# theovincent/i-DQN

Hardware: NVIDIA B200
Metric: i-DQN grad steps/sec (NatureCNN K=5, batch 32) (higher is better)
Workload: dtype f32

## Files before the change

i-dqn_b200/csrc/dense_wgrad_tma.cuh:

```cuda
#pragma once
#include "common.cuh"
#include "tc_core.cuh"
#include "tma_core.cuh"

namespace dwt {
using namespace tc;
typedef __nv_bfloat16 bf16;

constexpr int NTHREADS = 608;
constexpr int STAGES = 3;
constexpr int TM = 8;
constexpr int TN = 32;
constexpr int TO = 128;
constexpr int CB = 4;
constexpr uint32_t TILE_F32 = TM * CB * TO * 4;
constexpr uint32_t X_PLANE = 32 * TN * 2;
constexpr uint32_t STAGE_BYTES = 3 * TILE_F32 + 2 * X_PLANE;
constexpr uint32_t DY_CB = 2 * 2 * 32 * 128;
constexpr uint32_t DY_BYTES = CB * DY_CB;
constexpr uint32_t BAR_OFF = STAGES * STAGE_BYTES + DY_BYTES;
constexpr uint32_t SMEM_TOTAL = BAR_OFF + 256 + 1024;
constexpr uint32_t TMEM_COLS = 512;

struct Args {
  int heads, tile0, ntiles;
  int I, O;
  const int32_t* count;
  float lr, b1, b2, eps;
  float* grad;
  unsigned long long stream_policy;
  int64_t stride, w_off;
  int tl_id;
};

__device__ __forceinline__ void tma_store_3d(const CUtensorMap* map, uint32_t src, int c0, int c1, int c2) {
  asm volatile("cp.async.bulk.tensor.3d.global.shared::cta.bulk_group [%0, {%2, %3, %4}], [%1];" ::"l"(map), "r"(src),
               "r"(c0), "r"(c1), "r"(c2)
               : "memory");
}
__device__ __forceinline__ void bulk_commit() { asm volatile("cp.async.bulk.commit_group;" ::: "memory"); }
template <int N>
__device__ __forceinline__ void bulk_wait_read() {
  asm volatile("cp.async.bulk.wait_group.read %0;" ::"n"(N) : "memory");
}
__device__ __forceinline__ void bulk_wait_all() { asm volatile("cp.async.bulk.wait_group 0;" ::: "memory"); }
__device__ __forceinline__ void epi_bar_sync() { asm volatile("bar.sync 1, 512;" ::: "memory"); }

__global__ void __launch_bounds__(NTHREADS, 1)
dense_wgrad_adam_kernel(const __grid_constant__ CUtensorMap mapX_hi, const __grid_constant__ CUtensorMap mapX_lo,
                        const __grid_constant__ CUtensorMap mapDy_hi, const __grid_constant__ CUtensorMap mapDy_lo,
                        const __grid_constant__ CUtensorMap mapW, const __grid_constant__ CUtensorMap mapM,
                        const __grid_constant__ CUtensorMap mapV, const Args p) {
  extern __shared__ uint8_t smem_raw[];
  const uint32_t base = (smem_u32(smem_raw) + 1023u) & ~1023u;
  uint8_t* smem = smem_raw + (base - smem_u32(smem_raw));
  uint64_t* bars = reinterpret_cast<uint64_t*>(smem + BAR_OFF);
  uint64_t* full = bars;
  uint64_t* empty = bars + 4;
  uint64_t* acc_full = bars + 8;
  uint64_t* acc_empty = bars + 10;
  uint64_t* a_full = bars + 12;
  uint64_t* a_empty = bars + 13;
  uint64_t* ready = bars + 14;
  __shared__ uint32_t tmem_base_s;

  const int tid = threadIdx.x, warp = tid >> 5, lane = tid & 31;
  ktl_begin(p.tl_id);
  if (tid == 0) {
    for (int i = 0; i < STAGES; ++i) mbar_init(&full[i], 1), mbar_init(&empty[i], 1), mbar_init(&ready[i], 1);
    for (int i = 0; i < 2; ++i) mbar_init(&acc_full[i], 1), mbar_init(&acc_empty[i], 16);
    mbar_init(a_full, 1), mbar_init(a_empty, 1);
    fence_mbar_init();
  }
  if (warp == 1) tmem_alloc(&tmem_base_s, TMEM_COLS);
  fence_proxy_async_smem();
  tcgen05_before_sync();
  __syncthreads();
  tcgen05_after_sync();
  const uint32_t tmem = tmem_base_s;

  const int n_items = p.heads * p.ntiles;
  const int i0 = (int)((int64_t)blockIdx.x * n_items / gridDim.x), i1 = (int)((int64_t)(blockIdx.x + 1) * n_items / gridDim.x);
  const uint32_t as = base + STAGES * STAGE_BYTES;

  if (warp == 0) {
    if (elect_one()) {
      int st = 0, ai = 0, last_z = -1;
      uint32_t ph = 0;
      for (int it = i0; it < i1; ++it) {
        const int z = it / p.ntiles, row0 = (p.tile0 + it % p.ntiles) * TM;
        if (z != last_z) {
          last_z = z;
          mbar_wait(a_empty, (ai & 1) ^ 1);
          tma::expect_tx(a_full, DY_BYTES);
          for (int g = 0; g < 2 * CB; ++g) {
            const uint32_t dst = as + (g >> 1) * DY_CB + (g & 1) * 4096;
            tma::load_3d(dst, &mapDy_hi, a_full, g * 64, 0, z);
            tma::load_3d(dst + 8192, &mapDy_lo, a_full, g * 64, 0, z);
          }
          ++ai;
        }
        mbar_wait(&empty[st], ph ^ 1);
        tma::expect_tx(&full[st], STAGE_BYTES);
        const uint32_t s0 = base + st * STAGE_BYTES;
        tma::load_3d(s0 + 3 * TILE_F32, &mapX_hi, &full[st], row0, 0, z);
        tma::load_3d(s0 + 3 * TILE_F32 + X_PLANE, &mapX_lo, &full[st], row0, 0, z);
        for (int hb = 0; hb < 2; ++hb) {
          tma::load_3d_hint(s0 + hb * (TILE_F32 / 2), &mapW, &full[st], hb * 256, row0, z, p.stream_policy);
          tma::load_3d_hint(s0 + TILE_F32 + hb * (TILE_F32 / 2), &mapM, &full[st], hb * 256, row0, z, p.stream_policy);
          tma::load_3d_hint(s0 + 2 * TILE_F32 + hb * (TILE_F32 / 2), &mapV, &full[st], hb * 256, row0, z, p.stream_policy);
        }
        if (++st == STAGES) st = 0, ph ^= 1;
      }
    }
  } else if (warp == 1) {
    if (elect_one()) {
      const uint32_t idesc2 = make_idesc_bf16(128, 2 * TN, true, true);
      const uint32_t idesc1 = make_idesc_bf16(128, TN, true, true);
      const uint32_t a_hi32 = tma::desc_hi32(1024, tma::LT_SW128), b_hi32 = tma::desc_hi32(512, tma::LT_SW64);
      int st = 0, ai = 0, ti = 0, last_z = -1;
      uint32_t ph = 0;
      for (int it = i0; it < i1; ++it, ++ti) {
        const int z = it / p.ntiles;
        if (z != last_z) {
          last_z = z;
          mbar_wait(a_full, ai & 1);
          ++ai;
        }
        const int ab = ti & 1;
        mbar_wait(&acc_empty[ab], ((ti >> 1) & 1) ^ 1);
        mbar_wait(&full[st], ph);
        tcgen05_after_sync();
        const uint32_t xh = tma::desc_lo32(base + st * STAGE_BYTES + 3 * TILE_F32, X_PLANE);
#pragma unroll
        for (int cbk = 0; cbk < CB; ++cbk) {
          const uint32_t d = tmem + (uint32_t)ab * (CB * 2 * TN) + cbk * 2 * TN;
          const uint32_t ah = tma::desc_lo32(as + cbk * DY_CB, 4096), al = tma::desc_lo32(as + cbk * DY_CB + 8192, 4096);
          tma::mma_bf16_split<false>(d, ah, a_hi32, xh, b_hi32, idesc2);
          tma::mma_bf16_split<true>(d, al, a_hi32, xh, b_hi32, idesc1);
          tma::mma_bf16_split<true>(d, ah + 128, a_hi32, xh + 64, b_hi32, idesc2);
          tma::mma_bf16_split<true>(d, al + 128, a_hi32, xh + 64, b_hi32, idesc1);
        }
        mma_commit(&acc_full[ab]);
        if (it + 1 == i1 || (it + 1) / p.ntiles != z) mma_commit(a_empty);
        if (++st == STAGES) st = 0, ph ^= 1;
      }
    }
  } else if (warp == 18) {
    if (elect_one()) {
      int st = 0;
      uint32_t ph = 0;
      for (int it = i0; it < i1; ++it) {
        const int z = it / p.ntiles, row0 = (p.tile0 + it % p.ntiles) * TM;
        mbar_wait(&ready[st], ph);
        const uint32_t src = base + st * STAGE_BYTES;
        for (int hb = 0; hb < 2; ++hb) {
          tma::store_3d_hint(&mapW, src + hb * (TILE_F32 / 2), hb * 256, row0, z, p.stream_policy);
          tma::store_3d_hint(&mapM, src + TILE_F32 + hb * (TILE_F32 / 2), hb * 256, row0, z, p.stream_policy);
          tma::store_3d_hint(&mapV, src + 2 * TILE_F32 + hb * (TILE_F32 / 2), hb * 256, row0, z, p.stream_policy);
        }
        bulk_commit();
        bulk_wait_read<0>();
        tma::arrive(&empty[st]);
        if (++st == STAGES) st = 0, ph ^= 1;
      }
      bulk_wait_all();
    }
  } else {
    const int q = warp & 3, o = q * 32 + lane, cbk = (warp - 2) >> 2;
    int st = 0, ti = 0, last_z = -1;
    uint32_t ph = 0;
    AdamCoef ac;
    for (int it = i0; it < i1; ++it, ++ti) {
      const int z = it / p.ntiles, row0 = (p.tile0 + it % p.ntiles) * TM;
      if (z != last_z) {
        last_z = z;
        ac = adam_coef(p.b1, p.b2, p.lr, p.eps, p.count[z]);
      }
      const int ab = ti & 1;
      mbar_wait(&acc_full[ab], (ti >> 1) & 1);
      mbar_wait(&full[st], ph);
      tcgen05_after_sync();
      float g[16];
      {
        const uint32_t taddr = tmem + ((uint32_t)(q * 32) << 16) + (uint32_t)ab * (CB * 2 * TN) + cbk * 2 * TN;
        float g2[16];
        tmem_ld16_nowait(taddr, g);
        tmem_ld16_nowait(taddr + TN, g2);
        tmem_ld_wait();
#pragma unroll
        for (int e = 0; e < TM; ++e) g[e] += g2[e];
      }
      tcgen05_before_sync();
      __syncwarp();
      if (lane == 0) tma::arrive(&acc_empty[ab]);
      float* sW = reinterpret_cast<float*>(smem + st * STAGE_BYTES + (cbk >> 1) * (TILE_F32 / 2)) + (cbk & 1) * 128 + o;
      float* sM = sW + TILE_F32 / 4;
      float* sV = sM + TILE_F32 / 4;
      const int64_t gb = (int64_t)z * p.stride + p.w_off + (int64_t)row0 * p.O + cbk * 128 + o;
      float P[TM], M[TM], V[TM];
#pragma unroll
      for (int e = 0; e < TM; ++e) P[e] = sW[e * 256], M[e] = sM[e * 256], V[e] = sV[e * 256];
#pragma unroll
      for (int e = 0; e < TM; ++e) {
        adam_elem(ac, g[e], P[e], M[e], V[e]);
        sW[e * 256] = P[e], sM[e * 256] = M[e], sV[e * 256] = V[e];
      }
      fence_proxy_async_smem();
      epi_bar_sync();
      if (tid == 64) tma::arrive(&ready[st]);
      if (p.grad) {
#pragma unroll
        for (int e = 0; e < TM; ++e) p.grad[gb + (int64_t)e * p.O] = g[e];
      }
      if (++st == STAGES) st = 0, ph ^= 1;
    }
  }
  tcgen05_before_sync();
  __syncthreads();
  ktl_end(p.tl_id);
  if (warp == 1) tmem_dealloc(tmem, TMEM_COLS);
}

}
```

i-dqn_b200/csrc/img_host.cuh:

```cuda
#pragma once
#include "conv_img.cuh"
#include "dense_stream.cuh"
#include "dense_wgrad_tma.cuh"

struct ImgHost {
  img::Geom g[IDQN_IMG_LAYERS];
  img::TapsArgs fwd[IDQN_IMG_LAYERS], dg[IDQN_IMG_LAYERS];
  img::WgradArgs wg[IDQN_IMG_LAYERS];
  img::S2dArgs s2d;
  img::ChainArgs chain;
  int chain_on;
  int dense_on;
  alignas(64) CUtensorMap fmapWf[2], fmapWd, dmapX[2], dmapDy[2];
  alignas(64) CUtensorMap wmapX[2], wmapP[3];
  int wgrad_tma_on;
  dense::Args dfwd, ddg;
  float* dpart;
  int* dtickets;
};

static int img_chunks(int rows, int* chunk_rows, int* rows_alloc) {
  const int n = (rows + 255) / 256;
  int cr = ((rows + n - 1) / n + 7) / 8 * 8;
  *chunk_rows = cr;
// ... 471 lines not shown
  CK(cudaGetLastError());
  mark(h, dgrad ? "img_dgrad_L%d" : "img_fwd_L%d", li);
  return IDQN_OK;
}

static int img_launch_chain_fwd(idqn_handle* h) {
  ImgHost* H = (ImgHost*)h->img_host;
  img::ChainArgs c = H->chain;
  c.a.tl_id = tl_next(h);
  const img::ChainSmem L = img::chain_smem(c);
  const int per = (c.a.n_units + h->sm_avail - 1) / h->sm_avail;
  const int grid = (c.a.n_units + per - 1) / per;
  CK(img_set_smem(img::conv_chain_fwd_kernel, L.total));
  CK(launch_pdl(h->pdl, img::conv_chain_fwd_kernel, dim3(grid), dim3(img::NTHREADS), L.total, h->stream, h->il[1].mapX[0],
                h->il[1].mapX[1], h->il[1].mapW[0], h->il[1].mapW[1], h->il[2].mapW[0], h->il[2].mapW[1], c));
  CK(cudaGetLastError());
  mark(h, "img_fwd_chain_L%d", 1);
  return IDQN_OK;
}

static int img_launch_wgrad(idqn_handle* h, int li, int a_planes) {
  ImgHost* H = (ImgHost*)h->img_host;
  img::WgradArgs a = H->wg[li];
  a.debug = img_debug_on("wgrad", li);
  a.tl_id = tl_next(h);
  const ImgLayerState& S = h->il[li];
  const img::WgradSmem L = img::wgrad_smem(a, a_planes);
  const int grid = a.heads * a.groups * a.tsplit;
  if (a_planes == 1) {
    CK(img_set_smem(img::conv_wgrad_kernel<1>, L.total));
    CK(launch_pdl(h->pdl, img::conv_wgrad_kernel<1>, dim3(grid), dim3(img::WG_THREADS), L.total, h->stream, S.mapXw[0], S.mapXw[1],
                  S.mapZw[0], S.mapZw[1], a));
  } else {
    CK(img_set_smem(img::conv_wgrad_kernel<2>, L.total));
    CK(launch_pdl(h->pdl, img::conv_wgrad_kernel<2>, dim3(grid), dim3(img::WG_THREADS), L.total, h->stream, S.mapXw[0], S.mapXw[1],
                  S.mapZw[0], S.mapZw[1], a));
  }
  CK(cudaGetLastError());
  mark(h, "img_wgrad_L%d", li);
  return IDQN_OK;
}

static int dense_launch(idqn_handle* h, bool dgrad, bool z_dst, int unit0 = -1, int n_units = -1) {
  ImgHost* H = (ImgHost*)h->img_host;
  dense::Args a = dgrad ? H->ddg : H->dfwd;
  if (unit0 >= 0) a.unit0 = unit0, a.n_units = n_units;
  a.tl_id = unit0 >= 0 ? -1 : tl_next(h);
  const int li = IDQN_IMG_LAYERS;
  a.debug = img_debug_on(dgrad ? "ddgrad" : "dfwd", li);
  if (dgrad && z_dst) {
    const img::Geom& pg = H->g[li - 1];
    a.yh = h->il[li - 1].dz_hi, a.yl = h->il[li - 1].dz_lo;
    a.zP = pg.P, a.zW = pg.OW, a.zC = pg.OC, a.zOff = pg.T - 1, a.zRows = pg.ZRa, a.zstride = h->il[li - 1].dz_net_stride;
  }
  a.keep_heads = l2_keep_heads(h);
  const dense::Smem L = dense::smem_layout(a);
  int grid = std::min(a.n_units, h->sm_count);
  {
    static const bool rounds_env = !getenv("IDQN_NO_ROUNDS");
    if (rounds_env && unit0 < 0) {
      const int per = (a.n_units + grid - 1) / grid;
      grid = (a.n_units + per - 1) / per;
    }
  }
  if (dgrad) {
    CK(img_set_smem(dense::dense_stream_kernel<1>, L.total));
    CK(launch_pdl(h->pdl, dense::dense_stream_kernel<1>, dim3(grid), dim3(dense::NTHREADS), L.total, h->stream,
                  H->fmapWd, H->fmapWd, H->dmapDy[0], H->dmapDy[1], a));
  } else {
    CK(img_set_smem(dense::dense_stream_kernel<0>, L.total));
    CK(launch_pdl(h->pdl, dense::dense_stream_kernel<0>, dim3(grid), dim3(dense::NTHREADS), L.total, h->stream,
                  H->fmapWf[0], H->fmapWf[1], H->dmapX[0], H->dmapX[1], a));
  }
  CK(cudaGetLastError());
  mark(h, dgrad ? "dense_dgrad_L%d" : "dense_fwd_L%d", li);
  return IDQN_OK;
}

static int dense_wgrad_launch(idqn_handle* h, int tile0, int ntiles, bool keep_grads) {
  ImgHost* H = (ImgHost*)h->img_host;
  const Layer& l = h->layers[IDQN_IMG_LAYERS];
  dwt::Args a;
  a.heads = h->K, a.tile0 = tile0, a.ntiles = ntiles;
  a.I = l.g.Kd, a.O = l.g.OC;
  a.count = h->count;
  a.lr = h->cfg.learning_rate, a.b1 = 0.9f, a.b2 = 0.999f, a.eps = h->cfg.adam_eps;
  a.grad = keep_grads ? h->grad : nullptr;
  static const int sp = getenv("IDQN_L2_STREAM") ? atoi(getenv("IDQN_L2_STREAM")) : 0;
  a.stream_policy = sp == 0 ? tma::L2_EVICT_NORMAL : (sp == 2 ? tma::L2_EVICT_LAST : tma::L2_EVICT_FIRST);
  a.stride = h->stride, a.w_off = l.w_off;
  a.tl_id = tl_next(h);
  const int grid = std::min(a.heads * a.ntiles, h->sm_avail);
  CK(img_set_smem(dwt::dense_wgrad_adam_kernel, dwt::SMEM_TOTAL));
  CK(launch_pdl(0, dwt::dense_wgrad_adam_kernel, dim3(grid), dim3(dwt::NTHREADS), dwt::SMEM_TOTAL, h->stream, H->wmapX[0],
                H->wmapX[1], H->dmapDy[0], H->dmapDy[1], H->wmapP[0], H->wmapP[1], H->wmapP[2], a));
  CK(cudaGetLastError());
  mark(h, "dense_wgrad_adam_L%d", IDQN_IMG_LAYERS);
  return IDQN_OK;
}

static int img_rebuild_activation(idqn_handle* h, int net, int layer) {
  ImgHost* H = (ImgHost*)h->img_host;
  const img::Geom& g = H->g[layer];
  img::PlaneDst d = H->fwd[layer].dst;
  float* out = h->act + (int64_t)net * h->act_stride + h->layers[layer].act_off;
  const int64_t total = (int64_t)h->B * g.OH * g.OW * g.OC;
  img::planes_to_f32_kernel<<<(int)std::min<int64_t>((total + 255) / 256, 4096), 256, 0, h->stream>>>(d, net, h->B, g.OH, g.OW,
                                                                                                 g.OC, out);
  CK(cudaGetLastError());
  return IDQN_OK;
}
```

i-dqn_b200/csrc/net.cu:

```cuda
#include "common.cuh"
#include "gemm_simt.cuh"
#include "gemm_tc.cuh"
#include "sm_partition.cuh"

#include <algorithm>
#include <cmath>

static thread_local char g_err[512] = "";
void idqn_set_error(const char* fmt, ...) {
  va_list ap;
  va_start(ap, fmt);
  vsnprintf(g_err, sizeof(g_err), fmt, ap);
  va_end(ap);
}
extern "C" const char* idqn_last_error(void) { return g_err; }
extern "C" int idqn_version(void) { return 100; }

static void same_pad(int in, int k, int s, int* out, int* lo) {
  *out = (in + s - 1) / s;
  int total = std::max((*out - 1) * s + k - in, 0);
  *lo = total / 2;
}

static void finish_geom(ConvGeom& g) {
// ... 862 lines not shown
    tcg::TcDgradConv p;
    p.g = l.g;
    p.dyh = h->dact_hi + l.act_off, p.dyl = h->dact_lo + l.act_off, p.dystride = h->act_stride;
    p.wh = wh, p.wl = wl;
    p.w_off = l.w_off;
    p.xact = h->act + prev.act_off, p.dx = h->dact + prev.act_off;
    p.mask = mask, p.add = add;
    p.dxh = h->dact_hi + prev.act_off, p.dxl = h->dact_lo + prev.act_off, p.xstride = h->act_stride;
    p.ncls = S * S, p.JH = JH, p.JW = JW;
    p.d_jwoc = FastDiv(JW * l.g.OC);
    p.K = JH * JW * l.g.OC;
    p.NT = round16(l.g.IC);
    p.nstage = tcg::pick_stages(2, p.NT, (p.K + 31) / 32);
    for (int cl = 0; cl < p.ncls; ++cl) {
      p.cls_niy[cl] = cls_niy[cl], p.cls_nix[cl] = cls_nix[cl];
      p.cls_d_n[cl] = FastDiv(std::max(cls_niy[cl] * cls_nix[cl], 1));
      p.cls_d_nix[cl] = FastDiv(std::max(cls_nix[cl], 1));
    }
    dim3 grid((maxM + 127) / 128, 1, K * p.ncls);
    CK((tcg::launch_tc<false, false, 2, false, true, false>(p, grid, h->part, h->tickets, h->stream)));
    mark(h, "tc_dgrad_L%d", li);
    return IDQN_OK;
  }
  DgradProb p;
  p.g = l.g;
  p.dy = h->dact + l.act_off;
  p.dystride = h->act_stride;
  p.w = NetPtr{h->online, h->online, h->stride, h->stride, K};
  p.w_off = l.w_off;
  p.xact = h->act + prev.act_off;
  p.mask = mask, p.add = add;
  p.dx = h->dact + prev.act_off;
  p.dxh = h->dact_hi + prev.act_off, p.dxl = h->dact_lo + prev.act_off;
  p.xstride = h->act_stride;
  p.nz = K;
  p.S = 1;
  p.ncls = S * S;
  p.JH = JH, p.JW = JW;
  p.d_jwoc = FastDiv(JW * l.g.OC);
  p.N = l.g.IC;
  p.K = JH * JW * l.g.OC;
  p.kchunk = p.K;
  for (int cl = 0; cl < p.ncls; ++cl) {
    p.cls_niy[cl] = cls_niy[cl], p.cls_nix[cl] = cls_nix[cl];
    p.cls_d_n[cl] = FastDiv(std::max(cls_niy[cl] * cls_nix[cl], 1));
    p.cls_d_nix[cl] = FastDiv(std::max(cls_nix[cl], 1));
  }
  p.M = maxM;
  CK((launch_gemm_simt<true, true>(p, K * p.ncls, h->part, h->tickets, h->stream)));
  mark(h, "dgrad_L%d", li);
  return IDQN_OK;
}

static int launch_adam_ranges(idqn_handle* h, int64_t off_a, int64_t len_a, bool a_from_partials, int64_t off_b,
                              int64_t len_b, bool coresident = false) {
  len_a = std::max<int64_t>(len_a, 0), len_b = std::max<int64_t>(len_b, 0);
  if (len_a + len_b <= 0) return IDQN_OK;
  const int64_t n4a = len_a / 4, n4b = len_b / 4;
  const int cap = h->sm_count * 8;
  const int bt = coresident ? 128 : 256;
  const int ba = n4a ? (int)std::min<int64_t>((n4a + bt - 1) / bt, cap) : 0;
  const int bb = n4b ? (int)std::min<int64_t>((n4b + bt - 1) / bt, cap) : 0;
  if (coresident) {
    static bool carve_set = false;
    if (!carve_set) {
      CK(cudaFuncSetAttribute(adam_kernel, cudaFuncAttributePreferredSharedMemoryCarveout, cudaSharedmemCarveoutMaxShared));
      carve_set = true;
    }
  }
  dim3 grid(std::max(ba + bb, 1), h->K);
  const bool keep = (h->cfg.flags & IDQN_F_KEEP_GRADS) != 0;
  CK(launch_pdl(h->pdl && !coresident, adam_kernel, grid, dim3(bt), 0, h->stream, (float4*)h->online, (const float4*)h->grad, (float4*)h->mu, (float4*)h->nu,
                                           (uint2*)h->won_hi, (uint2*)h->won_lo, h->count, h->stride / 4, off_a / 4, n4a, ba,
                                           off_b / 4, n4b, h->cfg.learning_rate, 0.9f, 0.999f, h->cfg.adam_eps,
                                           a_from_partials ? (const float4*)h->wpart : nullptr, h->wgroups, h->wspan / 4,
                                           (a_from_partials && keep) ? (float4*)h->grad : nullptr, tl_next(h)));
  mark(h, "adam_%d", 0);
  return IDQN_OK;
}

static int dense_update_ctas(const idqn_handle* h) {
  static const int env = getenv("IDQN_WG_OVERLAP") ? atoi(getenv("IDQN_WG_OVERLAP")) : -1;
  if (h->update_ctas_set > 0) return std::min(h->sm_count, h->update_ctas_set - 1);
  return env >= 0 ? env : (h->K <= 10 ? std::min(h->sm_count, (116 + 13 * h->K) / 2 * h->sm_count / 148) : 0);
}

static int enqueue_learn_step(idqn_handle* h, int x_u8, bool dry = false, int64_t* ws_part = nullptr,
                              int* ws_tick = nullptr) {
  const int K = h->K, L = h->n_layers, B = h->B;
  h->n_launch = 0;
  const bool use_img = h->img_on && x_u8 && !dry;
  const int n_img = use_img ? IDQN_IMG_LAYERS : 0;
  if (!dry) h->img_last = use_img;
  const bool in_planes = use_tc(h) && (tc_conv_ok(h->layers[0]) || tc_dense_ok(h, h->layers[0]));
  if (use_img) {
    int rc = img_launch_s2d(h, x_u8);
    if (rc) return rc;
    const bool chain = ((ImgHost*)h->img_host)->chain_on && (h->cfg.flags & IDQN_F_CHAIN);
    for (int li = 0; li < n_img; ++li) {
      if (chain && li == 1) {
        rc = img_launch_chain_fwd(h);
        li = 2;
      } else {
        rc = img_launch_taps(h, li, false, li == 0 ? 1 : 2);
      }
      if (rc) return rc;
    }
  } else if (in_planes && !dry) {
    int rc = launch_input_planes(h, x_u8, B, 1);
    if (rc) return rc;
  }
  const int64_t in_full = (int64_t)B * h->in_elems;
  const bool use_dense = h->img_on && !dry && ((ImgHost*)h->img_host)->dense_on;
  for (int li = n_img; li < L - 1; ++li) {
    if (use_dense && li == IDQN_IMG_LAYERS) {
      int rc = dense_launch(h, false, false);
      if (rc) return rc;
      continue;
    }
    FwdIO io;
    int nh = 1;
    if (li == 0) {
      io.x = NetPtr{h->s, h->s2, 0, 0, K};
      io.xh = NetPtr{h->in_hi, h->in_hi + in_full, 0, 0, K};
      io.xl = NetPtr{h->in_lo, h->in_lo + in_full, 0, 0, K};
      nh = K;
    } else {
      const int64_t o = h->layers[li - 1].act_off;
      io.x = NetPtr{h->act + o, h->act + o, h->act_stride, h->act_stride, 2 * K};
      io.xh = NetPtr{h->act_hi + o, h->act_hi + o, h->act_stride, h->act_stride, 2 * K};
      io.xl = NetPtr{h->act_lo + o, h->act_lo + o, h->act_stride, h->act_stride, 2 * K};
    }
    io.w = NetPtr{h->online, h->target, h->stride, h->stride, K};
    io.wh = NetPtr{h->won_hi, h->wtg_hi, h->stride, h->stride, K};
    io.wl = NetPtr{h->won_lo, h->wtg_lo, h->stride, h->stride, K};
    const int64_t o = h->layers[li].act_off;
    io.y = h->act + o, io.yh = h->act_hi + o, io.yl = h->act_lo + o, io.ystride = h->act_stride;
    if (h->layers[li].kind == IDQN_LAYER_POOL) {
      if (dry) continue;
      int rc = launch_pool_fwd(h, li, 2 * K, B, h->act + h->layers[li - 1].act_off, h->act + o, h->act_stride, true);
      if (rc) return rc;
      continue;
    }
    int rc = launch_fwd_layer(h, li, 2 * K, nh, B, io, li == 0 ? x_u8 : 0, h->layers[li].relu_out, dry, ws_part, ws_tick);
    if (rc) return rc;
  }
  if (!dry) {
    const Layer& l = h->layers[L - 1];
    HeadArgs a;
    if (L >= 2) {
      const float* hid = h->act + h->layers[L - 2].act_off;
      a.hid = NetPtr{hid, hid, h->act_stride, h->act_stride, 2 * K};
      a.dhid = h->dact + h->layers[L - 2].act_off;
      a.dhid_hi = h->dact_hi + h->layers[L - 2].act_off, a.dhid_lo = h->dact_lo + h->layers[L - 2].act_off;
      a.relu_mask = 1;
    } else {
      REQUIRE(!x_u8, "a network without hidden layers needs float32 inputs");
      a.hid = NetPtr{h->s, h->s2, 0, 0, K};
      a.dhid = nullptr;
      a.dhid_hi = a.dhid_lo = nullptr;
      a.relu_mask = 0;
    }
    a.H = l.g.Kd, a.A = h->A, a.B = B, a.K = K;
    a.online = h->online, a.target = h->target;
    a.stride = h->stride, a.w_off = l.w_off, a.b_off = l.b_off;
    a.action = h->action, a.reward = h->reward, a.terminal = h->terminal;
    a.gamma_n = h->cfg.gamma_n;
// ... 953 lines not shown
```

i-dqn_b200/csrc/tc_core.cuh:

```cuda
#pragma once
#include <cuda_bf16.h>
#include <cuda_runtime.h>
#include <stdint.h>

namespace tc {

__device__ __forceinline__ uint32_t smem_u32(const void* p) { return (uint32_t)__cvta_generic_to_shared(p); }

__device__ __forceinline__ void mbar_init(uint64_t* bar, uint32_t count) {
  asm volatile("mbarrier.init.shared::cta.b64 [%0], %1;" ::"r"(smem_u32(bar)), "r"(count) : "memory");
}
__device__ __forceinline__ void fence_mbar_init() { asm volatile("fence.mbarrier_init.release.cluster;" ::: "memory"); }
__device__ __forceinline__ bool mbar_try_wait(uint64_t* bar, uint32_t parity) {
  uint32_t ok;
  asm volatile(
      "{\n"
      ".reg .pred p;\n"
      "mbarrier.try_wait.parity.shared::cta.b64 p, [%1], %2;\n"
      "selp.u32 %0, 1, 0, p;\n"
      "}\n"
      : "=r"(ok)
      : "r"(smem_u32(bar)), "r"(parity)
      : "memory");
  return ok != 0;
}
__device__ __forceinline__ void mbar_wait(uint64_t* bar, uint32_t parity) {
  uint32_t spins = 0;
  while (!mbar_try_wait(bar, parity)) {
    if (++spins > (1u << 24)) __trap();
  }
}

__device__ __forceinline__ bool elect_one() {
  uint32_t pred = 0, laneid = 0;
  asm volatile(
      "{\n"
      ".reg .b32 %%rx;\n"
      ".reg .pred %%px;\n"
      "     elect.sync %%rx|%%px, %2;\n"
      "@%%px mov.s32 %1, 1;\n"
      "     mov.s32 %0, %%rx;\n"
      "}\n"
      : "+r"(laneid), "+r"(pred)
      : "r"(0xFFFFFFFF));
  return pred != 0;
}

__device__ __forceinline__ void fence_proxy_async_smem() { asm volatile("fence.proxy.async.shared::cta;" ::: "memory"); }
__device__ __forceinline__ void tcgen05_before_sync() { asm volatile("tcgen05.fence::before_thread_sync;" ::: "memory"); }
__device__ __forceinline__ void tcgen05_after_sync() { asm volatile("tcgen05.fence::after_thread_sync;" ::: "memory"); }

__device__ __forceinline__ void tmem_alloc(uint32_t* smem_dst, uint32_t ncols) {
  __syncwarp();
  asm volatile("tcgen05.alloc.cta_group::1.sync.aligned.shared::cta.b32 [%0], %1;" ::"r"(smem_u32(smem_dst)), "r"(ncols)
               : "memory");
  asm volatile("tcgen05.relinquish_alloc_permit.cta_group::1.sync.aligned;" ::: "memory");
}
__device__ __forceinline__ void tmem_dealloc(uint32_t taddr, uint32_t ncols) {
  __syncwarp();
  asm volatile("tcgen05.dealloc.cta_group::1.sync.aligned.b32 %0, %1;" ::"r"(taddr), "r"(ncols) : "memory");
}
__device__ __forceinline__ void tmem_ld16(uint32_t taddr, float* v) {
  uint32_t r[16];
  __syncwarp();
  asm volatile(
      "tcgen05.ld.sync.aligned.32x32b.x16.b32 {%0,%1,%2,%3,%4,%5,%6,%7,%8,%9,%10,%11,%12,%13,%14,%15}, [%16];"
      : "=r"(r[0]), "=r"(r[1]), "=r"(r[2]), "=r"(r[3]), "=r"(r[4]), "=r"(r[5]), "=r"(r[6]), "=r"(r[7]), "=r"(r[8]),
        "=r"(r[9]), "=r"(r[10]), "=r"(r[11]), "=r"(r[12]), "=r"(r[13]), "=r"(r[14]), "=r"(r[15])
      : "r"(taddr)
      : "memory");
  asm volatile("tcgen05.wait::ld.sync.aligned;" ::: "memory");
#pragma unroll
  for (int i = 0; i < 16; ++i) v[i] = __uint_as_float(r[i]);
}

__device__ __forceinline__ void tmem_ld16_nowait(uint32_t taddr, float* v) {
  uint32_t r[16];
  __syncwarp();
  asm volatile(
      "tcgen05.ld.sync.aligned.32x32b.x16.b32 {%0,%1,%2,%3,%4,%5,%6,%7,%8,%9,%10,%11,%12,%13,%14,%15}, [%16];"
      : "=r"(r[0]), "=r"(r[1]), "=r"(r[2]), "=r"(r[3]), "=r"(r[4]), "=r"(r[5]), "=r"(r[6]), "=r"(r[7]), "=r"(r[8]),
        "=r"(r[9]), "=r"(r[10]), "=r"(r[11]), "=r"(r[12]), "=r"(r[13]), "=r"(r[14]), "=r"(r[15])
      : "r"(taddr)
      : "memory");
#pragma unroll
  for (int i = 0; i < 16; ++i) v[i] = __uint_as_float(r[i]);
}
__device__ __forceinline__ void tmem_ld_wait() { asm volatile("tcgen05.wait::ld.sync.aligned;" ::: "memory"); }

__device__ __forceinline__ uint64_t make_smem_desc(uint32_t saddr, uint32_t lbo_bytes, uint32_t sbo_bytes) {
  uint64_t d = 0;
  d |= (uint64_t)((saddr >> 4) & 0x3FFFu);
  d |= (uint64_t)((lbo_bytes >> 4) & 0x3FFFu) << 16;
  d |= (uint64_t)((sbo_bytes >> 4) & 0x3FFFu) << 32;
  d |= (uint64_t)1 << 46;
  return d;
}
__host__ __device__ constexpr uint32_t make_idesc_bf16(int M, int N, bool a_mn_major, bool b_mn_major) {
  return (1u << 4)
         | (1u << 7)
         | (1u << 10)
         | ((a_mn_major ? 1u : 0u) << 15)
         | ((b_mn_major ? 1u : 0u) << 16)
         | ((uint32_t)(N >> 3) << 17)
         | ((uint32_t)(M >> 4) << 24);
}

__device__ __forceinline__ void mma_bf16(uint32_t d_tmem, uint64_t adesc, uint64_t bdesc, uint32_t idesc,
                                         uint32_t accumulate) {
  asm volatile(
      "{\n"
      ".reg .pred p;\n"
      "setp.ne.b32 p, %4, 0;\n"
      "tcgen05.mma.cta_group::1.kind::f16 [%0], %1, %2, %3, p;\n"
      "}\n" ::"r"(d_tmem),
      "l"(adesc), "l"(bdesc), "r"(idesc), "r"(accumulate)
      : "memory");
}
__device__ __forceinline__ void mma_commit(uint64_t* bar) {
  asm volatile("tcgen05.commit.cta_group::1.mbarrier::arrive::one.shared::cluster.b64 [%0];" ::"r"(smem_u32(bar))
               : "memory");
}

__device__ __forceinline__ void split8(const float* x, uint4& hi, uint4& lo) {
  uint32_t h[4], l[4];
#pragma unroll
  for (int i = 0; i < 4; ++i) {
    const __nv_bfloat162 hp = __floats2bfloat162_rn(x[2 * i], x[2 * i + 1]);
    const uint32_t hb = *reinterpret_cast<const uint32_t*>(&hp);
    const float r0 = x[2 * i] - __uint_as_float(hb << 16);
    const float r1 = x[2 * i + 1] - __uint_as_float(hb & 0xffff0000u);
    const __nv_bfloat162 lp = __floats2bfloat162_rn(r0, r1);
    h[i] = hb;
    l[i] = *reinterpret_cast<const uint32_t*>(&lp);
  }
  hi = make_uint4(h[0], h[1], h[2], h[3]);
  lo = make_uint4(l[0], l[1], l[2], l[3]);
}
__device__ __forceinline__ uint4 pack8_exact(const float* x) {
  uint32_t h[4];
#pragma unroll
  for (int i = 0; i < 4; ++i) {
    const __nv_bfloat162 hp = __floats2bfloat162_rn(x[2 * i], x[2 * i + 1]);
    h[i] = *reinterpret_cast<const uint32_t*>(&hp);
  }
  return make_uint4(h[0], h[1], h[2], h[3]);
}

__device__ __forceinline__ void split4(const float4& x, uint2& hi, uint2& lo) {
  const __nv_bfloat162 h0 = __floats2bfloat162_rn(x.x, x.y), h1 = __floats2bfloat162_rn(x.z, x.w);
  const uint32_t b0 = *reinterpret_cast<const uint32_t*>(&h0), b1 = *reinterpret_cast<const uint32_t*>(&h1);
  const __nv_bfloat162 l0 = __floats2bfloat162_rn(x.x - __uint_as_float(b0 << 16), x.y - __uint_as_float(b0 & 0xffff0000u));
  const __nv_bfloat162 l1 = __floats2bfloat162_rn(x.z - __uint_as_float(b1 << 16), x.w - __uint_as_float(b1 & 0xffff0000u));
  hi = make_uint2(b0, b1);
  lo = make_uint2(*reinterpret_cast<const uint32_t*>(&l0), *reinterpret_cast<const uint32_t*>(&l1));
}
__device__ __forceinline__ void st1_planes(__nv_bfloat16* hi, __nv_bfloat16* lo, float v) {
  const __nv_bfloat16 h = __float2bfloat16_rn(v);
  *hi = h;
  *lo = __float2bfloat16_rn(v - __bfloat162float(h));
}

struct AdamCoef {
  float b1, b2, omb1, omb2, rbc1, rbc2, lr, eps;
};
__device__ __forceinline__ AdamCoef adam_coef(float b1, float b2, float lr, float eps, int count) {
  AdamCoef c;
  const float t = (float)count;
  c.b1 = b1, c.b2 = b2, c.omb1 = 1.f - b1, c.omb2 = 1.f - b2;
// ... 31 lines not shown
```

i-dqn_b200/csrc/tma_core.cuh:

```cuda
#pragma once
#include <cuda.h>
#include <cuda_runtime.h>
#include <stdint.h>

#include "tc_core.cuh"

namespace tma {
using tc::smem_u32;

__device__ __forceinline__ void prefetch_desc(const CUtensorMap* m) {
  asm volatile("prefetch.tensormap [%0];" ::"l"(m) : "memory");
}
__device__ __forceinline__ void expect_tx(uint64_t* bar, uint32_t bytes) {
  asm volatile("mbarrier.arrive.expect_tx.shared::cta.b64 _, [%0], %1;" ::"r"(smem_u32(bar)), "r"(bytes) : "memory");
}
__device__ __forceinline__ void arrive(uint64_t* bar) {
  asm volatile("mbarrier.arrive.shared::cta.b64 _, [%0];" ::"r"(smem_u32(bar)) : "memory");
}
__device__ __forceinline__ void load_2d(uint32_t dst, const CUtensorMap* map, uint64_t* bar, int c0, int c1) {
  asm volatile(
      "cp.async.bulk.tensor.2d.shared::cluster.global.mbarrier::complete_tx::bytes [%0], [%1, {%3, %4}], [%2];" ::"r"(dst),
      "l"(map), "r"(smem_u32(bar)), "r"(c0), "r"(c1)
      : "memory");
}
__device__ __forceinline__ void load_3d(uint32_t dst, const CUtensorMap* map, uint64_t* bar, int c0, int c1, int c2) {
  asm volatile(
      "cp.async.bulk.tensor.3d.shared::cluster.global.mbarrier::complete_tx::bytes [%0], [%1, {%3, %4, %5}], [%2];" ::"r"(
          dst),
      "l"(map), "r"(smem_u32(bar)), "r"(c0), "r"(c1), "r"(c2)
      : "memory");
}
__device__ __forceinline__ void load_4d(uint32_t dst, const CUtensorMap* map, uint64_t* bar, int c0, int c1, int c2,
                                        int c3) {
  asm volatile(
      "cp.async.bulk.tensor.4d.shared::cluster.global.mbarrier::complete_tx::bytes [%0], [%1, {%3, %4, %5, %6}], [%2];" ::
          "r"(dst),
      "l"(map), "r"(smem_u32(bar)), "r"(c0), "r"(c1), "r"(c2), "r"(c3)
      : "memory");
}

constexpr uint64_t L2_EVICT_NORMAL = 0x1000000000000000ull, L2_EVICT_FIRST = 0x12F0000000000000ull,
                   L2_EVICT_LAST = 0x14F0000000000000ull;
__device__ __forceinline__ void load_3d_hint(uint32_t dst, const CUtensorMap* map, uint64_t* bar, int c0, int c1, int c2,
                                             uint64_t policy) {
  asm volatile(
      "cp.async.bulk.tensor.3d.shared::cluster.global.mbarrier::complete_tx::bytes.L2::cache_hint [%0], [%1, {%3, %4, %5}], "
      "[%2], %6;" ::"r"(dst),
      "l"(map), "r"(smem_u32(bar)), "r"(c0), "r"(c1), "r"(c2), "l"(policy)
      : "memory");
}
__device__ __forceinline__ void store_3d_hint(const CUtensorMap* map, uint32_t src, int c0, int c1, int c2, uint64_t policy) {
  asm volatile("cp.async.bulk.tensor.3d.global.shared::cta.bulk_group.L2::cache_hint [%0, {%2, %3, %4}], [%1], %5;" ::"l"(map),
               "r"(src), "r"(c0), "r"(c1), "r"(c2), "l"(policy)
               : "memory");
}
__device__ __forceinline__ void st1_planes_hint(__nv_bfloat16* hi, __nv_bfloat16* lo, float v, uint64_t policy) {
  const __nv_bfloat16 h = __float2bfloat16_rn(v);
  const __nv_bfloat16 l = __float2bfloat16_rn(v - __bfloat162float(h));
  asm volatile("st.global.L2::cache_hint.b16 [%0], %1, %2;" ::"l"(hi), "h"(*reinterpret_cast<const unsigned short*>(&h)), "l"(policy) : "memory");
  asm volatile("st.global.L2::cache_hint.b16 [%0], %1, %2;" ::"l"(lo), "h"(*reinterpret_cast<const unsigned short*>(&l)), "l"(policy) : "memory");
}

constexpr uint32_t LT_SW128 = 2, LT_SW64 = 4;
__device__ __forceinline__ uint64_t make_desc(uint32_t saddr, uint32_t lbo_bytes, uint32_t sbo_bytes, uint32_t layout_type) {
  uint64_t d = 0;
  d |= (uint64_t)((saddr >> 4) & 0x3FFFu);
  d |= (uint64_t)((lbo_bytes >> 4) & 0x3FFFu) << 16;
  d |= (uint64_t)((sbo_bytes >> 4) & 0x3FFFu) << 32;
  d |= (uint64_t)1 << 46;
  d |= (uint64_t)(layout_type & 7u) << 61;
  return d;
}

__device__ __forceinline__ uint32_t desc_hi32(uint32_t sbo_bytes, uint32_t layout_type) {
  return ((sbo_bytes >> 4) & 0x3FFFu) | (1u << 14) | ((layout_type & 7u) << 29);
}
__device__ __forceinline__ uint32_t desc_lo32(uint32_t saddr, uint32_t lbo_bytes) {
  return ((saddr >> 4) & 0x3FFFu) | (((lbo_bytes >> 4) & 0x3FFFu) << 16);
}
template <bool ACC>
__device__ __forceinline__ void mma_bf16_split(uint32_t d_tmem, uint32_t a_lo, uint32_t a_hi, uint32_t b_lo, uint32_t b_hi,
                                               uint32_t idesc) {
  if (ACC) {
    asm volatile(
        "{\n"
        ".reg .pred p;\n"
        ".reg .b64 da, db;\n"
        "setp.eq.u32 p, 1, 1;\n"
        "mov.b64 da, {%1, %2};\n"
        "mov.b64 db, {%3, %4};\n"
        "tcgen05.mma.cta_group::1.kind::f16 [%0], da, db, %5, p;\n"
        "}\n" ::"r"(d_tmem),
        "r"(a_lo), "r"(a_hi), "r"(b_lo), "r"(b_hi), "r"(idesc)
        : "memory");
  } else {
    asm volatile(
        "{\n"
        ".reg .pred p;\n"
        ".reg .b64 da, db;\n"
        "setp.ne.u32 p, 1, 1;\n"
        "mov.b64 da, {%1, %2};\n"
        "mov.b64 db, {%3, %4};\n"
        "tcgen05.mma.cta_group::1.kind::f16 [%0], da, db, %5, p;\n"
        "}\n" ::"r"(d_tmem),
        "r"(a_lo), "r"(a_hi), "r"(b_lo), "r"(b_hi), "r"(idesc)
        : "memory");
  }
}

typedef CUresult (*EncodeTiledFn)(CUtensorMap*, CUtensorMapDataType, cuuint32_t, void*, const cuuint64_t*,
                                  const cuuint64_t*, const cuuint32_t*, const cuuint32_t*, CUtensorMapInterleave,
                                  CUtensorMapSwizzle, CUtensorMapL2promotion, CUtensorMapFloatOOBfill);
static inline EncodeTiledFn encode_fn() {
  static EncodeTiledFn fn = nullptr;
  if (!fn) {
    void* p = nullptr;
    cudaDriverEntryPointQueryResult q;
    if (cudaGetDriverEntryPoint("cuTensorMapEncodeTiled", &p, cudaEnableDefault, &q) == cudaSuccess) fn = (EncodeTiledFn)p;
  }
  return fn;
}
static inline bool encode_f32(CUtensorMap* map, const void* base, int rank, const uint64_t* dims, const uint64_t* strides,
                              const uint32_t* box) {
  EncodeTiledFn fn = encode_fn();
  if (!fn) return false;
  cuuint64_t gd[5], gs[5];
  cuuint32_t bx[5], es[5];
  for (int i = 0; i < rank; ++i) gd[i] = dims[i], bx[i] = box[i], es[i] = 1;
  for (int i = 0; i + 1 < rank; ++i) gs[i] = strides[i];
  return fn(map, CU_TENSOR_MAP_DATA_TYPE_FLOAT32, (cuuint32_t)rank, const_cast<void*>(base), gd, gs, bx, es,
            CU_TENSOR_MAP_INTERLEAVE_NONE, CU_TENSOR_MAP_SWIZZLE_NONE, CU_TENSOR_MAP_L2_PROMOTION_L2_256B,
            CU_TENSOR_MAP_FLOAT_OOB_FILL_NONE) == CUDA_SUCCESS;
}
static inline bool encode_bf16(CUtensorMap* map, const void* base, int rank, const uint64_t* dims, const uint64_t* strides,
                               const uint32_t* box, int sw_bytes) {
  EncodeTiledFn fn = encode_fn();
  if (!fn) return false;
// ... 12 lines not shown
```

Baseline: 3620.

## Replace TMA store warp with direct epilogue stores and split X barrier

The dedicated TMA-store warp and the named barrier across epilogue warps are removed. Eight epilogue warps now alternate between the two accumulator buffers, and each warp handles two column blocks. Each warp reads W/M/V from shared memory, releases the stage early, and writes the Adam results straight to global memory with L2 cache-hint stores. X loads get their own barrier, so the MMA can start before the large W/M/V tiles arrive. The CTA-count heuristic for overlapping the dense update is also retuned. This trades bulk TMA stores for per-thread coalesced stores and may increase LSU pressure.

```diff
diff --git a/i-dqn_b200/csrc/dense_wgrad_tma.cuh b/i-dqn_b200/csrc/dense_wgrad_tma.cuh
--- a/i-dqn_b200/csrc/dense_wgrad_tma.cuh
+++ b/i-dqn_b200/csrc/dense_wgrad_tma.cuh
@@ -7,12 +7,14 @@
 using namespace tc;
 typedef __nv_bfloat16 bf16;
 
-constexpr int NTHREADS = 608;
+constexpr int NTHREADS = 576;
+constexpr int EPI_WARPS = 8;
 constexpr int STAGES = 3;
 constexpr int TM = 8;
 constexpr int TN = 32;
 constexpr int TO = 128;
 constexpr int CB = 4;
+constexpr int O = CB * TO;
 constexpr uint32_t TILE_F32 = TM * CB * TO * 4;
 constexpr uint32_t X_PLANE = 32 * TN * 2;
 constexpr uint32_t STAGE_BYTES = 3 * TILE_F32 + 2 * X_PLANE;
@@ -24,27 +26,19 @@
 
 struct Args {
   int heads, tile0, ntiles;
-  int I, O;
+  int I;
   const int32_t* count;
   float lr, b1, b2, eps;
   float* grad;
+  float *w, *mu, *nu;
   unsigned long long stream_policy;
   int64_t stride, w_off;
   int tl_id;
 };
 
-__device__ __forceinline__ void tma_store_3d(const CUtensorMap* map, uint32_t src, int c0, int c1, int c2) {
-  asm volatile("cp.async.bulk.tensor.3d.global.shared::cta.bulk_group [%0, {%2, %3, %4}], [%1];" ::"l"(map), "r"(src),
-               "r"(c0), "r"(c1), "r"(c2)
-               : "memory");
+__device__ __forceinline__ void st_f32_hint(float* dst, float v, uint64_t policy) {
+  asm volatile("st.global.L2::cache_hint.f32 [%0], %1, %2;" ::"l"(dst), "f"(v), "l"(policy) : "memory");
 }
-__device__ __forceinline__ void bulk_commit() { asm volatile("cp.async.bulk.commit_group;" ::: "memory"); }
-template <int N>
-__device__ __forceinline__ void bulk_wait_read() {
-  asm volatile("cp.async.bulk.wait_group.read %0;" ::"n"(N) : "memory");
-}
-__device__ __forceinline__ void bulk_wait_all() { asm volatile("cp.async.bulk.wait_group 0;" ::: "memory"); }
-__device__ __forceinline__ void epi_bar_sync() { asm volatile("bar.sync 1, 512;" ::: "memory"); }
 
 __global__ void __launch_bounds__(NTHREADS, 1)
 dense_wgrad_adam_kernel(const __grid_constant__ CUtensorMap mapX_hi, const __grid_constant__ CUtensorMap mapX_lo,
@@ -61,14 +55,14 @@
   uint64_t* acc_empty = bars + 10;
   uint64_t* a_full = bars + 12;
   uint64_t* a_empty = bars + 13;
-  uint64_t* ready = bars + 14;
+  uint64_t* xfull = bars + 14;
   __shared__ uint32_t tmem_base_s;
 
   const int tid = threadIdx.x, warp = tid >> 5, lane = tid & 31;
   ktl_begin(p.tl_id);
   if (tid == 0) {
-    for (int i = 0; i < STAGES; ++i) mbar_init(&full[i], 1), mbar_init(&empty[i], 1), mbar_init(&ready[i], 1);
-    for (int i = 0; i < 2; ++i) mbar_init(&acc_full[i], 1), mbar_init(&acc_empty[i], 16);
+    for (int i = 0; i < STAGES; ++i) mbar_init(&full[i], 1), mbar_init(&empty[i], EPI_WARPS), mbar_init(&xfull[i], 1);
+    for (int i = 0; i < 2; ++i) mbar_init(&acc_full[i], 1), mbar_init(&acc_empty[i], EPI_WARPS);
     mbar_init(a_full, 1), mbar_init(a_empty, 1);
     fence_mbar_init();
   }
@@ -101,10 +95,11 @@
           ++ai;
         }
         mbar_wait(&empty[st], ph ^ 1);
-        tma::expect_tx(&full[st], STAGE_BYTES);
         const uint32_t s0 = base + st * STAGE_BYTES;
-        tma::load_3d(s0 + 3 * TILE_F32, &mapX_hi, &full[st], row0, 0, z);
-        tma::load_3d(s0 + 3 * TILE_F32 + X_PLANE, &mapX_lo, &full[st], row0, 0, z);
+        tma::expect_tx(&xfull[st], 2 * X_PLANE);
+        tma::load_3d(s0 + 3 * TILE_F32, &mapX_hi, &xfull[st], row0, 0, z);
+        tma::load_3d(s0 + 3 * TILE_F32 + X_PLANE, &mapX_lo, &xfull[st], row0, 0, z);
+        tma::expect_tx(&full[st], 3 * TILE_F32);
         for (int hb = 0; hb < 2; ++hb) {
           tma::load_3d_hint(s0 + hb * (TILE_F32 / 2), &mapW, &full[st], hb * 256, row0, z, p.stream_policy);
           tma::load_3d_hint(s0 + TILE_F32 + hb * (TILE_F32 / 2), &mapM, &full[st], hb * 256, row0, z, p.stream_policy);
@@ -129,7 +124,7 @@
         }
         const int ab = ti & 1;
         mbar_wait(&acc_empty[ab], ((ti >> 1) & 1) ^ 1);
-        mbar_wait(&full[st], ph);
+        mbar_wait(&xfull[st], ph);
         tcgen05_after_sync();
         const uint32_t xh = tma::desc_lo32(base + st * STAGE_BYTES + 3 * TILE_F32, X_PLANE);
 #pragma unroll
@@ -146,74 +141,70 @@
         if (++st == STAGES) st = 0, ph ^= 1;
       }
     }
-  } else if (warp == 18) {
-    if (elect_one()) {
-      int st = 0;
-      uint32_t ph = 0;
-      for (int it = i0; it < i1; ++it) {
-        const int z = it / p.ntiles, row0 = (p.tile0 + it % p.ntiles) * TM;
-        mbar_wait(&ready[st], ph);
-        const uint32_t src = base + st * STAGE_BYTES;
-        for (int hb = 0; hb < 2; ++hb) {
-          tma::store_3d_hint(&mapW, src + hb * (TILE_F32 / 2), hb * 256, row0, z, p.stream_policy);
-          tma::store_3d_hint(&mapM, src + TILE_F32 + hb * (TILE_F32 / 2), hb * 256, row0, z, p.stream_policy);
-          tma::store_3d_hint(&mapV, src + 2 * TILE_F32 + hb * (TILE_F32 / 2), hb * 256, row0, z, p.stream_policy);
-        }
-        bulk_commit();
-        bulk_wait_read<0>();
-        tma::arrive(&empty[st]);
-        if (++st == STAGES) st = 0, ph ^= 1;
-      }
-      bulk_wait_all();
-    }
   } else {
-    const int q = warp & 3, o = q * 32 + lane, cbk = (warp - 2) >> 2;
-    int st = 0, ti = 0, last_z = -1;
+    const int q = warp & 3, o = q * 32 + lane, gr = (warp - 2) >> 3, cbh = ((warp - 2) >> 2) & 1;
+    int z = i0 / p.ntiles, t = i0 % p.ntiles, st = 0, ti = 0, last_z = -1;
     uint32_t ph = 0;
     AdamCoef ac;
     for (int it = i0; it < i1; ++it, ++ti) {
-      const int z = it / p.ntiles, row0 = (p.tile0 + it % p.ntiles) * TM;
-      if (z != last_z) {
-        last_z = z;
-        ac = adam_coef(p.b1, p.b2, p.lr, p.eps, p.count[z]);
-      }
-      const int ab = ti & 1;
-      mbar_wait(&acc_full[ab], (ti >> 1) & 1);
-      mbar_wait(&full[st], ph);
-      tcgen05_after_sync();
-      float g[16];
-      {
-        const uint32_t taddr = tmem + ((uint32_t)(q * 32) << 16) + (uint32_t)ab * (CB * 2 * TN) + cbk * 2 * TN;
-        float g2[16];
-        tmem_ld16_nowait(taddr, g);
-        tmem_ld16_nowait(taddr + TN, g2);
-        tmem_ld_wait();
-#pragma unroll
-        for (int e = 0; e < TM; ++e) g[e] += g2[e];
-      }
-      tcgen05_before_sync();
-      __syncwarp();
-      if (lane == 0) tma::arrive(&acc_empty[ab]);
-      float* sW = reinterpret_cast<float*>(smem + st * STAGE_BYTES + (cbk >> 1) * (TILE_F32 / 2)) + (cbk & 1) * 128 + o;
-      float* sM = sW + TILE_F32 / 4;
-      float* sV = sM + TILE_F32 / 4;
-      const int64_t gb = (int64_t)z * p.stride + p.w_off + (int64_t)row0 * p.O + cbk * 128 + o;
-      float P[TM], M[TM], V[TM];
-#pragma unroll
-      for (int e = 0; e < TM; ++e) P[e] = sW[e * 256], M[e] = sM[e * 256], V[e] = sV[e * 256];
-#pragma unroll
-      for (int e = 0; e < TM; ++e) {
-        adam_elem(ac, g[e], P[e], M[e], V[e]);
-        sW[e * 256] = P[e], sM[e * 256] = M[e], sV[e * 256] = V[e];
-      }
-      fence_proxy_async_smem();
-      epi_bar_sync();
-      if (tid == 64) tma::arrive(&ready[st]);
-      if (p.grad) {
-#pragma unroll
-        for (int e = 0; e < TM; ++e) p.grad[gb + (int64_t)e * p.O] = g[e];
+      if ((ti & 1) == gr) {
+        const int row0 = (p.tile0 + t) * TM;
+        if (z != last_z) {
+          last_z = z;
+          ac = adam_coef(p.b1, p.b2, p.lr, p.eps, p.count[z]);
+        }
+        mbar_wait(&acc_full[gr], (ti >> 1) & 1);
+        mbar_wait(&full[st], ph);
+        tcgen05_after_sync();
+        float g[2][TM];
+        {
+          const uint32_t taddr = tmem + ((uint32_t)(q * 32) << 16) + (uint32_t)gr * (CB * 2 * TN) + 2 * cbh * 2 * TN;
+          float g2[2][TM];
+#pragma unroll
+          for (int j = 0; j < 2; ++j) {
+            tmem_ld8_nowait(taddr + j * 2 * TN, g[j]);
+            tmem_ld8_nowait(taddr + j * 2 * TN + TN, g2[j]);
+          }
+          tmem_ld_wait();
+#pragma unroll
+          for (int j = 0; j < 2; ++j)
+#pragma unroll
+            for (int e = 0; e < TM; ++e) g[j][e] += g2[j][e];
+        }
+        tcgen05_before_sync();
+        __syncwarp();
+        if (lane == 0) tma::arrive(&acc_empty[gr]);
+        const float* sW = reinterpret_cast<const float*>(smem + st * STAGE_BYTES + cbh * (TILE_F32 / 2)) + o;
+        const float* sM = sW + TILE_F32 / 4;
+        const float* sV = sM + TILE_F32 / 4;
+        float P[2][TM], M[2][TM], V[2][TM];
+#pragma unroll
+        for (int j = 0; j < 2; ++j)
+#pragma unroll
+          for (int e = 0; e < TM; ++e)
+            P[j][e] = sW[e * 256 + j * 128], M[j][e] = sM[e * 256 + j * 128], V[j][e] = sV[e * 256 + j * 128];
+        fence_proxy_async_smem();
+        __syncwarp();
+        if (lane == 0) tma::arrive(&empty[st]);
+#pragma unroll
+        for (int j = 0; j < 2; ++j) {
+          const int64_t gb = (int64_t)z * p.stride + p.w_off + (int64_t)row0 * O + (2 * cbh + j) * TO + o;
+          float *gw = p.w + gb, *gm = p.mu + gb, *gv = p.nu + gb;
+#pragma unroll
+          for (int e = 0; e < TM; ++e) {
+            adam_elem(ac, g[j][e], P[j][e], M[j][e], V[j][e]);
+            st_f32_hint(gw + e * O, P[j][e], p.stream_policy);
+            st_f32_hint(gm + e * O, M[j][e], p.stream_policy);
+            st_f32_hint(gv + e * O, V[j][e], p.stream_policy);
+          }
+          if (p.grad) {
+#pragma unroll
+            for (int e = 0; e < TM; ++e) p.grad[gb + e * O] = g[j][e];
+          }
+        }
       }
       if (++st == STAGES) st = 0, ph ^= 1;
+      if (++t == p.ntiles) t = 0, ++z;
     }
   }
   tcgen05_before_sync();
diff --git a/i-dqn_b200/csrc/img_host.cuh b/i-dqn_b200/csrc/img_host.cuh
--- a/i-dqn_b200/csrc/img_host.cuh
+++ b/i-dqn_b200/csrc/img_host.cuh
@@ -577,10 +577,11 @@
   const Layer& l = h->layers[IDQN_IMG_LAYERS];
   dwt::Args a;
   a.heads = h->K, a.tile0 = tile0, a.ntiles = ntiles;
-  a.I = l.g.Kd, a.O = l.g.OC;
+  a.I = l.g.Kd;
   a.count = h->count;
   a.lr = h->cfg.learning_rate, a.b1 = 0.9f, a.b2 = 0.999f, a.eps = h->cfg.adam_eps;
   a.grad = keep_grads ? h->grad : nullptr;
+  a.w = h->online, a.mu = h->mu, a.nu = h->nu;
   static const int sp = getenv("IDQN_L2_STREAM") ? atoi(getenv("IDQN_L2_STREAM")) : 0;
   a.stream_policy = sp == 0 ? tma::L2_EVICT_NORMAL : (sp == 2 ? tma::L2_EVICT_LAST : tma::L2_EVICT_FIRST);
   a.stride = h->stride, a.w_off = l.w_off;
diff --git a/i-dqn_b200/csrc/net.cu b/i-dqn_b200/csrc/net.cu
--- a/i-dqn_b200/csrc/net.cu
+++ b/i-dqn_b200/csrc/net.cu
@@ -968,7 +968,7 @@
 static int dense_update_ctas(const idqn_handle* h) {
   static const int env = getenv("IDQN_WG_OVERLAP") ? atoi(getenv("IDQN_WG_OVERLAP")) : -1;
   if (h->update_ctas_set > 0) return std::min(h->sm_count, h->update_ctas_set - 1);
-  return env >= 0 ? env : (h->K <= 10 ? std::min(h->sm_count, (116 + 13 * h->K) / 2 * h->sm_count / 148) : 0);
+  return env >= 0 ? env : (h->K <= 10 ? std::min(h->sm_count, (58 + 4 * h->K) * h->sm_count / 148) : 0);
 }
 
 static int enqueue_learn_step(idqn_handle* h, int x_u8, bool dry = false, int64_t* ws_part = nullptr,
diff --git a/i-dqn_b200/csrc/tc_core.cuh b/i-dqn_b200/csrc/tc_core.cuh
--- a/i-dqn_b200/csrc/tc_core.cuh
+++ b/i-dqn_b200/csrc/tc_core.cuh
@@ -85,6 +85,16 @@
       : "memory");
 #pragma unroll
   for (int i = 0; i < 16; ++i) v[i] = __uint_as_float(r[i]);
+}
+__device__ __forceinline__ void tmem_ld8_nowait(uint32_t taddr, float* v) {
+  uint32_t r[8];
+  __syncwarp();
+  asm volatile("tcgen05.ld.sync.aligned.32x32b.x8.b32 {%0,%1,%2,%3,%4,%5,%6,%7}, [%8];"
+               : "=r"(r[0]), "=r"(r[1]), "=r"(r[2]), "=r"(r[3]), "=r"(r[4]), "=r"(r[5]), "=r"(r[6]), "=r"(r[7])
+               : "r"(taddr)
+               : "memory");
+#pragma unroll
+  for (int i = 0; i < 8; ++i) v[i] = __uint_as_float(r[i]);
 }
 __device__ __forceinline__ void tmem_ld_wait() { asm volatile("tcgen05.wait::ld.sync.aligned;" ::: "memory"); }
 
diff --git a/i-dqn_b200/csrc/tma_core.cuh b/i-dqn_b200/csrc/tma_core.cuh
--- a/i-dqn_b200/csrc/tma_core.cuh
+++ b/i-dqn_b200/csrc/tma_core.cuh
@@ -48,11 +48,6 @@
       "[%2], %6;" ::"r"(dst),
       "l"(map), "r"(smem_u32(bar)), "r"(c0), "r"(c1), "r"(c2), "l"(policy)
       : "memory");
-}
-__device__ __forceinline__ void store_3d_hint(const CUtensorMap* map, uint32_t src, int c0, int c1, int c2, uint64_t policy) {
-  asm volatile("cp.async.bulk.tensor.3d.global.shared::cta.bulk_group.L2::cache_hint [%0, {%2, %3, %4}], [%1], %5;" ::"l"(map),
-               "r"(src), "r"(c0), "r"(c1), "r"(c2), "l"(policy)
-               : "memory");
 }
 __device__ __forceinline__ void st1_planes_hint(__nv_bfloat16* hi, __nv_bfloat16* lo, float v, uint64_t policy) {
   const __nv_bfloat16 h = __float2bfloat16_rn(v);
```

New measurement: 3702 (median of 6 runs). 1.02x the previous value.
